# ChaissonLab/LRA

Hardware: AMD Instinct MI355X
Metric: aligned Gbp/s, 30 kb ONT vs GRCh38 (MapRead_lowacc end to end incl. SAM text), per job (higher is better)
Workload: dtype int32

## Files before the change

lra_amd/csrc/indel_refine.hip:

```cpp
#include "common.h"
#include "scan.h"
#include <algorithm>
#include <stdlib.h>

int lra_aog_launch_device(lra_ctx* ctx, int n, const char* d_qseq, const char* d_tseq, const uint64_t* d_q_off,
                          const int32_t* d_q_len, const uint64_t* d_t_off, const int32_t* d_t_len, const int32_t* d_k,
                          int m, int mm, int indel, int32_t* d_score, int32_t* d_nblocks, int32_t* d_blocks,
                          const uint64_t* d_block_off, int32_t* d_status);

namespace {

constexpr int BAD = -999999999;
constexpr int NEG = -2000000000;
enum { C_DIAG = 0, C_LEFT = 1, C_DOWN = 2, C_BOUND = 3, C_DELCLOSE = 4, C_INSCLOSE = 5, C_DONE = 6 };

__device__ __forceinline__ void wave_sync() {
  __builtin_amdgcn_fence(__ATOMIC_RELEASE, "workgroup");
  __builtin_amdgcn_wave_barrier();
  __builtin_amdgcn_fence(__ATOMIC_ACQUIRE, "workgroup");
}

__device__ __forceinline__ void wave_sync_lds() {
  __builtin_amdgcn_fence(__ATOMIC_RELEASE, "wavefront");
  __builtin_amdgcn_wave_barrier();
// ... 87 lines not shown
        qStart += advanced; tStart += advanced;
      }
      long ll = el;
      if (el > maxGap) {
        usedAlt = true;
        altQ = eq + maxGap; altT = et + maxGap; altL = el - maxGap;
        ll = maxGap;
        qPos = eq + maxGap; tPos = et + maxGap;
      }
      const long qEnd = eq + ll, tEnd = et + ll;
      const long tLen = tPos - tStart;
      const long tSeqLen = tEnd - tStart, qSeqLen = qEnd - qStart;
      const bool aog = (tSeqLen < k || qSeqLen < k);
      if (EMIT) {
        const uint64_t s = so + nseg;
        A.s_aln[s] = a; A.s_kind[s] = aog ? 1 : 0;
        A.s_qStart[s] = (int)qStart; A.s_tStart[s] = (int)tStart; A.s_qEnd[s] = (int)qEnd; A.s_tEnd[s] = (int)tEnd;
        A.s_b0[s] = (int)startBlock; A.s_b1[s] = (int)endBlock;
        A.s_first[3 * s] = (int)fq; A.s_first[3 * s + 1] = (int)ft; A.s_first[3 * s + 2] = (int)fl;
        A.s_lastLen[s] = (int)ll;
        A.s_rows[s] = aog ? 0 : (uint64_t)(tLen > 0 ? tLen : 0);
        A.s_isAog[s] = aog ? 1u : 0u;
        A.i_kind[io + nitem] = 1; A.i_data[3 * (io + nitem)] = (int)(nseg);
      }
      nitem++; nseg++;
    }
    if (!usedAlt) endBlock++;
    else { ovIdx = endBlock; ovQ = altQ; ovT = altT; ovL = altL; }
    startBlock = endBlock;
  }
  if (!EMIT) { A.a_nseg[a] = nseg; A.a_nitem[a] = nitem; A.a_status[a] = 0; }
}

struct __attribute__((aligned(16))) Row { int S, E; unsigned int C; int T; };

constexpr int CB = 32;
constexpr int MAXW = 1024;

struct BandArgs {
  uint64_t n_seg, n_task;
  const int32_t* s_aln; const int32_t* s_kind; const int32_t* s_qStart; const int32_t* s_qEnd; const int32_t* s_tStart;
  const int32_t* s_b0; const int32_t* s_b1; const int32_t* s_first; const int32_t* s_lastLen;
  const uint64_t* s_rows; const uint64_t* s_row_off;
  const int32_t* ab; const uint64_t* block_off;
  const char* tseq; const uint64_t* t_off;
  int k;
  Row* rows;
  uint64_t* s_cells; int32_t* s_status; int32_t* s_width; uint64_t* s_tmpcap;
  uint32_t* s_nchunk; const uint64_t* chunk_off; uint32_t* task_seg; int32_t* chunkT; int32_t* chunkQ;
};

struct SegBlocks {
  const int32_t* ab; long b0, b1; int fq, ft, fl, lastLen;
  __device__ __forceinline__ void get(long b, long& q, long& t, long& l) const {
    if (b == b0) { q = fq; t = ft; l = fl; }
    else { q = ab[3 * b]; t = ab[3 * b + 1]; l = (b == b1) ? lastLen : ab[3 * b + 2]; }
  }
};
__device__ __forceinline__ SegBlocks seg_blocks(const BandArgs& B, uint64_t s) {
  SegBlocks v;
  const int a = B.s_aln[s];
  v.ab = B.ab + 3 * (B.block_off[a] + 2 * (uint64_t)a);
  v.b0 = B.s_b0[s]; v.b1 = B.s_b1[s];
  v.fq = B.s_first[3 * s]; v.ft = B.s_first[3 * s + 1]; v.fl = B.s_first[3 * s + 2]; v.lastLen = B.s_lastLen[s];
  return v;
}
struct BlockStep { int bqGap, btGap; long blockLength, rows, advq; };
__device__ __forceinline__ BlockStep block_step(const SegBlocks& sb, long b, long bq, long bt, long bl, long& nq2, long& nt2, long& nl2) {
  BlockStep st; st.bqGap = 0; st.btGap = 0; st.blockLength = bl; nq2 = nt2 = nl2 = 0;
  if (b < sb.b1) {
    sb.get(b + 1, nq2, nt2, nl2);
    st.bqGap = (int)(nq2 - (bq + bl)); st.btGap = (int)(nt2 - (bt + bl));
    if (st.bqGap > 0 && st.btGap > 0) { int c = min(st.bqGap, st.btGap); st.bqGap -= c; st.btGap -= c; st.blockLength += c; }
  }
  const long body = st.blockLength > 0 ? st.blockLength : 0;
  st.rows = body + (st.btGap > st.bqGap && st.btGap > 0 ? st.btGap : 0);
  st.advq = body + (st.bqGap > st.btGap && st.bqGap > 0 ? st.bqGap : 0);
  return st;
}

// ... 109 lines not shown
      flush(tOff - k);
    }
    if (st.bqGap > st.btGap) {
      for (int qi = 0; qi < st.bqGap; qi++, q++)
        for (int ki = 0; ki < k; ki++) {
          if (tOff - ki >= 0 && tOff - ki < tLen) { if (RG(ringE, tOff - ki) < q) RG(ringE, tOff - ki) = (int)q; }
          if (tOff + ki < tLen) { int v = RG(ringS, tOff + ki); if (v == 0 || v > q) RG(ringS, tOff + ki) = (int)q; }
        }
    }
    if (st.btGap > st.bqGap) {
      for (int ti = 0; ti < st.btGap; ti++) {
        if (tOff >= tLen) { status |= 1; break; }
        const int e = (int)min(qEnd - 1, q + k);
        RG(ringS, tOff) = (int)max(q - k, qStart); RG(ringE, tOff) = e;
        if (e < eMin) eMin = e;
        if (sHi < tOff) sHi = tOff;
        tOff++;
        flush(tOff - k);
      }
    }
    bq = nq2; bt = nt2; bl = nl2;
  }
  if (lastChunk) for (long r = max(0L, tOff - k + 1); r < tLen; r++) flush(r);
#undef RG
  if (!multi) { if (tOff != tLen) status |= 1; B.s_status[s] = status; }
}

__global__ void __launch_bounds__(64) ir_band_scan(BandArgs B) {
  const uint64_t s = blockIdx.x;
  const int lane = threadIdx.x;
  if (B.s_kind[s] != 0) { if (lane == 0) { B.s_cells[s] = 0; B.s_status[s] = 0; B.s_width[s] = 0; B.s_tmpcap[s] = 0; } return; }
  int status = B.s_status[s];
  const long tLen = (long)B.s_rows[s];
  Row* rows = B.rows + B.s_row_off[s];
  unsigned long long cells = 0;
  int width = 0;
  if (!status && tLen > 0) {
    int run = 0x7fffffff;
    for (long base = ((tLen - 1) / 64) * 64; base >= 0; base -= 64) {
      const long r = base + lane;
      const int own = (r < tLen) ? rows[r].S : 0x7fffffff;
      int v = own;
      for (int d = 1; d < 64; d <<= 1) { int o = __shfl_down(v, d); if (lane + d < 64) v = min(v, o); }
      v = min(v, run);
      if (r < tLen && v != own) rows[r].S = v;
      run = __shfl(v, 0);
    }
    const int a = B.s_aln[s];
    const unsigned char* tb = (const unsigned char*)B.tseq + B.t_off[a] + B.s_tStart[s];
    int runE = -0x7fffffff;
    for (long base = 0; base < tLen; base += 64) {
      const long r = base + lane;
      Row w; w.S = 0; w.E = -0x7fffffff; w.C = 0; w.T = 0;
      if (r < tLen) w = rows[r];
      int e = w.E;
      for (int d = 1; d < 64; d <<= 1) { int o = __shfl_up(e, d); if (lane >= d) e = max(e, o); }
      e = max(e, runE);
      runE = __shfl(e, 63);
      int len = (r < tLen) ? e - w.S + 1 : 0;
      if (r < tLen) {
        if (len < 1 || w.S < 0) status |= 1;
        else if (len > MAXW) status |= 4;
        width = max(width, len);
      }
      const unsigned long long l = (unsigned long long)max(len, 0);
      unsigned long long inc = l;
      for (int d = 1; d < 64; d <<= 1) { unsigned long long o = __shfl_up(inc, d); if (lane >= d) inc += o; }
      if (r < tLen) { w.E = e; w.C = (unsigned int)(cells + inc - l); w.T = tb[r]; rows[r] = w; }
      cells += __shfl(inc, 63);
    }
    for (int o = 32; o > 0; o >>= 1) { status |= __shfl_xor(status, o); width = max(width, __shfl_xor(width, o)); }
  }
  if (lane == 0) {
    B.s_cells[s] = status ? 0 : cells;
    B.s_status[s] = status;
    B.s_width[s] = status ? 0 : width;
    B.s_tmpcap[s] = status ? 0 : (uint64_t)(tLen + ((long)B.s_qEnd[s] - B.s_qStart[s]) + 2);
  }
}

constexpr int FILL_BINS = 128;
template <bool EMIT>
__global__ void ir_classify(uint64_t n_seg, const int32_t* __restrict__ s_kind, const int32_t* __restrict__ s_status, const int32_t* __restrict__ s_width,
                            const uint64_t* __restrict__ s_rows, int* bins, uint32_t* list) {
  const uint64_t s = (uint64_t)blockIdx.x * blockDim.x + threadIdx.x;
  const int lane = threadIdx.x & 63;
  int bin = -1;
  if (s < n_seg && s_kind[s] == 0 && s_status[s] == 0) {
    const int w = s_width[s];
    const uint32_t r = (uint32_t)min((unsigned long long)s_rows[s], 0x7fffffffULL);
    bin = (w <= 16 ? 0 : w <= 32 ? 1 : w <= 64 ? 2 : 3) * 32 + (r ? __clz(r) : 31);
  }
  const unsigned long long below = (lane == 0) ? 0ULL : (~0ULL >> (64 - lane));
  unsigned long long todo = __ballot(bin >= 0);
  while (todo) {
    const int leader = __ffsll((long long)todo) - 1;
    const int b = __shfl(bin, leader);
    const unsigned long long m = __ballot(bin == b);
    int base = 0;
    if (lane == leader) base = atomicAdd(&bins[b], __popcll(m));
    base = __shfl(base, leader);
    if (EMIT && bin == b) list[base + __popcll(m & below)] = (uint32_t)s;
// ... 7 lines not shown
  const Row* rows;
  const char* qseq; const uint64_t* q_off; const int32_t* q_len;
  int match, mismatch, g;
  unsigned char* path;
  const uint32_t* list; int* cursor;
};

__device__ __forceinline__ bool is_bound(long row, int c, int len) { return c == len - 1 || (row > 0 && c == 0); }

__device__ __forceinline__ int shr1(int x, int fill) { return __builtin_amdgcn_update_dpp(fill, x, 0x138, 0xf, 0xf, false); }
template <int G>
__device__ __forceinline__ int scan_max(int w) {
  w = max(w, __builtin_amdgcn_update_dpp(NEG, w, 0x111, 0xf, 0xf, false));
  w = max(w, __builtin_amdgcn_update_dpp(NEG, w, 0x112, 0xf, 0xf, false));
  w = max(w, __builtin_amdgcn_update_dpp(NEG, w, 0x114, 0xf, 0xf, false));
  w = max(w, __builtin_amdgcn_update_dpp(NEG, w, 0x118, 0xf, 0xf, false));
  if (G >= 32) w = max(w, __builtin_amdgcn_update_dpp(NEG, w, 0x142, 0xa, 0xf, false));
  if (G >= 64) w = max(w, __builtin_amdgcn_update_dpp(NEG, w, 0x143, 0xc, 0xf, false));
  return w;
}

template <int G>
__global__ void __launch_bounds__(64) ir_fill(FillArgs F) {
  constexpr int GP = 64 / G;
  constexpr int CLS = (G == 16) ? 0 : (G == 32) ? 1 : 2;
  const int lane = threadIdx.x;
  const int c = lane % G, gbase = lane - c;
  const int g = F.g, go = 2 * F.g + 1;
  const long listEnd = F.cursor[4 + CLS];
  const uint32_t* list = F.list;
  long ti = -1, tLen = 0;
  const Row* rows = nullptr; const unsigned char* qb = nullptr; unsigned char* P = nullptr;
  long chunkBase = 0, qLast = 0;
  Row chunk; chunk.S = chunk.E = chunk.T = 0; chunk.C = 0;
  int W0 = 0, qlo = 0, qhi = 0, qnext = 0;
  int prevM = BAD, prevD = BAD, prevS = 0, prevLen = 0;
  bool done = false;
  auto ldq = [&](long idx) -> int { return qb[idx < qLast ? idx : qLast]; };
  while (true) {
    if (!done && ti < 0) {
      long x = 0;
      if (c == 0) x = atomicAdd(&F.cursor[CLS], 1);
      x = __shfl(x, gbase);
      if (x < listEnd) {
        const uint64_t s = list[x];
        const int a = F.s_aln[s];
        tLen = (long)F.s_rows[s];
        rows = F.rows + F.s_row_off[s];
        qb = (const unsigned char*)F.qseq + F.q_off[a];
        qLast = (long)F.q_len[a] - 1;
        P = F.path + F.s_cell_off[s];
        ti = 0; chunkBase = 0;
        if (c < tLen) chunk = rows[c];
        W0 = rows[0].S;
        qlo = ldq((long)W0 + c); qhi = ldq((long)W0 + G + c); qnext = ldq((long)W0 + 2 * G + c);
      } else done = true;
    }
    if (__ballot(!done) == 0ULL) break;
    if (!done && ti - chunkBase == G) { chunkBase = ti; if (ti + c < tLen) chunk = rows[ti + c]; }
    const int src = gbase + (int)((ti - chunkBase) & (G - 1));
    const int S = __shfl(chunk.S, src), E = __shfl(chunk.E, src), tch = __shfl(chunk.T, src);
    const unsigned int C = __shfl(chunk.C, src);
    while (!done && S - W0 >= G) { W0 += G; qlo = qhi; qhi = qnext; qnext = ldq((long)W0 + 2 * G + c); }
    const int j = S - W0 + c;
    const int q1 = __shfl(qlo, gbase + (j & (G - 1))), q2 = __shfl(qhi, gbase + (j & (G - 1)));
    const int qch = (j < G) ? q1 : q2;
    const int len = E - S + 1;
    const bool lastRow = (ti == tLen - 1);
    const int off = S - prevS;
    const bool interior = c >= 1 && (lastRow ? c <= len - 1 : c <= len - 2);
    const int srcA = c + off, srcD = srcA - 1;
    const bool aboveIn = srcA <= prevLen - 1;
    const int aM = __shfl(prevM, gbase + (srcA & (G - 1))), aD = __shfl(prevD, gbase + (srcA & (G - 1)));
    const int dM = shr1(aM, BAD);
    const bool okA = aboveIn && !is_bound(ti - 1, srcA, prevLen);
    const bool okD = aboveIn && srcD >= 0 && !is_bound(ti - 1, srcD, prevLen);
    const int dOpen = okA ? aM + go : BAD, dExt = okA ? aD : BAD;
    const int Dv = max(dOpen, dExt);
    const int delOpen = (Dv == dOpen) ? 1 : 0;
    const int mS = okD ? dM + (tch == qch ? F.match : F.mismatch) : BAD;
    const int dS = okA ? aM + g : BAD;
    const int V = interior ? max(mS, max(dS, Dv)) : NEG;
    const int W = scan_max<G>(V);
    int Wm1 = shr1(W, NEG), Vm1 = shr1(V, NEG);
    if (c == 0) { Wm1 = NEG; Vm1 = NEG; }
    const int Iv = max(BAD, go + Wm1);
    int M = max(max(BAD, V), max(Vm1 + g, go + Wm1));
    if (!interior) M = BAD;
    int Mleft = shr1(M, BAD);
    if (c <= 1) Mleft = BAD;
    const int iOpen = Mleft + go;
    const int insOpen = (Iv == iOpen) ? 1 : 0;
    const int iS = Mleft + g;
    int code;
    if (!interior) code = C_BOUND;
    else if (M == mS) code = C_DIAG;
    else if (M == iS) code = C_LEFT;
    else if (M == dS) code = C_DOWN;
    else if (M == Dv) code = C_DELCLOSE;
    else code = C_INSCLOSE;
    int outM = M, outD = interior ? Dv : BAD;
    unsigned char outB = (unsigned char)(code | (delOpen << 3) | (insOpen << 4));
    if (ti == 0) {
      const bool last0 = (c == len - 1) && (tLen > 1);
      outM = last0 ? BAD : (c == 0 ? 0 : c * g);
      outD = BAD;
      outB = (unsigned char)(last0 ? C_BOUND : (c == 0 ? C_DONE : C_LEFT));
    }
    if (!done) {
      if (c < len) P[C + c] = outB;
      prevM = outM; prevD = outD; prevS = S; prevLen = len;
      ti++;
      if (ti == tLen) ti = -1;
    }
  }
}


__global__ void __launch_bounds__(64) ir_fill_wide(FillArgs F) {
  __shared__ int sM[2][MAXW + 64], sD[2][MAXW + 64];
  const int lane = threadIdx.x;
  const int g = F.g, go = 2 * F.g + 1;
  const long listEnd = F.cursor[4 + 3];
  while (true) {
    long x = 0;
    if (lane == 0) x = atomicAdd(&F.cursor[3], 1);
    x = (long)(((unsigned long long)(unsigned)__builtin_amdgcn_readfirstlane((int)((unsigned long long)x >> 32)) << 32) | (unsigned)__builtin_amdgcn_readfirstlane((int)(x & 0xffffffffL)));
    if (x >= listEnd) break;
    const uint64_t s = F.list[x];
    const int a = F.s_aln[s];
    const long tLen = (long)F.s_rows[s];
    const Row* rows = F.rows + F.s_row_off[s];
    const unsigned char* qb = (const unsigned char*)F.qseq + F.q_off[a];
    const long qLast = (long)F.q_len[a] - 1;
    unsigned char* P = F.path + F.s_cell_off[s];
    int prevS = 0, prevLen = 0;
    for (long ti = 0; ti < tLen; ti++) {
      const Row rw = rows[ti];
      const int S = rw.S, len = rw.E - rw.S + 1, tch = rw.T;
      const unsigned int C = rw.C;
      const bool lastRow = (ti == tLen - 1);
      const int off = S - prevS;
      const int cur = (int)(ti & 1), prv = cur ^ 1;
      int carryW = NEG, carryV = NEG, carryM = BAD;
      for (int base = 0; base < len; base += 64) {
        const int c = base + lane;
        int outM, outD; unsigned char outB;
        if (ti == 0) {
          const bool last0 = (c == len - 1) && (tLen > 1);
          outM = last0 ? BAD : (c == 0 ? 0 : c * g);
          outD = BAD;
          outB = (unsigned char)(last0 ? C_BOUND : (c == 0 ? C_DONE : C_LEFT));
        } else {
          const long qi = (long)S + c;
          const int qch = qb[qi < qLast ? qi : qLast];
          const bool interior = c >= 1 && (lastRow ? c <= len - 1 : c <= len - 2);
          const int srcA = c + off, srcD = srcA - 1;
          const bool aboveIn = srcA <= prevLen - 1;
          const bool inA = srcA >= 0 && srcA < prevLen, inD = srcD >= 0 && srcD < prevLen;
          const int aM = inA ? sM[prv][srcA] : BAD, aD = inA ? sD[prv][srcA] : BAD;
          const int dM = inD ? sM[prv][srcD] : BAD;
          const bool okA = aboveIn && !is_bound(ti - 1, srcA, prevLen);
          const bool okD = aboveIn && srcD >= 0 && !is_bound(ti - 1, srcD, prevLen);
          const int dOpen = okA ? aM + go : BAD, dExt = okA ? aD : BAD;
          const int Dv = max(dOpen, dExt);
          const int delOpen = (Dv == dOpen) ? 1 : 0;
          const int mS = okD ? dM + (tch == qch ? F.match : F.mismatch) : BAD;
          const int dS = okA ? aM + g : BAD;
          const int V = interior ? max(mS, max(dS, Dv)) : NEG;
          const int W = max(scan_max<64>(V), carryW);
          int Wm1 = shr1(W, NEG), Vm1 = shr1(V, NEG);
          if (lane == 0) { Wm1 = carryW; Vm1 = carryV; }
          if (c == 0) { Wm1 = NEG; Vm1 = NEG; }
          const int Iv = max(BAD, go + Wm1);
          int M = max(max(BAD, V), max(Vm1 + g, go + Wm1));
          if (!interior) M = BAD;
          int Mleft = shr1(M, BAD);
          if (lane == 0) Mleft = carryM;
          if (c <= 1) Mleft = BAD;
          const int iOpen = Mleft + go;
          const int insOpen = (Iv == iOpen) ? 1 : 0;
          const int iS = Mleft + g;
          int code;
          if (!interior) code = C_BOUND;
          else if (M == mS) code = C_DIAG;
          else if (M == iS) code = C_LEFT;
          else if (M == dS) code = C_DOWN;
          else if (M == Dv) code = C_DELCLOSE;
          else code = C_INSCLOSE;
          outM = M; outD = interior ? Dv : BAD;
          outB = (unsigned char)(code | (delOpen << 3) | (insOpen << 4));
          carryW = __shfl(W, 63); carryV = __shfl(V, 63); carryM = __shfl(M, 63);
        }
        if (c < len) { P[C + c] = outB; sM[cur][c] = outM; sD[cur][c] = outD; }
      }
      wave_sync_lds();
      prevS = S; prevLen = len;
    }
  }
}

template <int N>
__device__ __forceinline__ int ror(int x) { return __builtin_amdgcn_update_dpp(0, x, 0x120 + N, 0xf, 0xf, true); }
__device__ __forceinline__ int pin(int x) { asm volatile("" : "+v"(x)); return x; }
__device__ __forceinline__ int ring_scan_max(int w, int d) {
  { const int t = pin(max(w, ror<1>(w))); w = (d >= 1) ? t : w; }
  { const int t = pin(max(w, ror<2>(w))); w = (d >= 2) ? t : w; }
  { const int t = pin(max(w, ror<4>(w))); w = (d >= 4) ? t : w; }
  { const int t = pin(max(w, ror<8>(w))); w = (d >= 8) ? t : w; }
  return w;
}
template <int NP>
__global__ void __launch_bounds__(64) ir_fill_cols(FillArgs F) {
  constexpr int G = 16;
  constexpr int CLS = NP - 1;
  const int lane = threadIdx.x;
  const int c = lane % G, gbase = lane - c;
  const int g = F.g, go = 2 * F.g + 1;
  const long listEnd = F.cursor[4 + CLS];
  const uint32_t* list = F.list;
  long ti = -1, tLen = 0;
  const Row* rows = nullptr; const unsigned char* qb = nullptr; unsigned char* P = nullptr;
  long qLast = 0;
  __shared__ Row s_chunk[64];
  long chunkBase = 0;
  Row chunk; chunk.S = chunk.E = chunk.T = 0; chunk.C = 0;
  int K0 = 0, q0 = 0, q1 = 0, q2 = 0, q3 = 0;
  int pM[NP], pD[NP], prevS = 0, prevLen = 0;
  for (int p = 0; p < NP; p++) { pM[p] = BAD; pD[p] = BAD; }
  bool done = false;
  auto ldq = [&](long idx) -> int { return qb[idx < qLast ? idx : qLast]; };
  while (true) {
    if (!done && ti < 0) {
      long x = 0;
      if (c == 0) x = atomicAdd(&F.cursor[CLS], 1);
      x = __shfl(x, gbase);
      if (x < listEnd) {
        const uint64_t s = list[x];
        const int a = F.s_aln[s];
        tLen = (long)F.s_rows[s];
        rows = F.rows + F.s_row_off[s];
        qb = (const unsigned char*)F.qseq + F.q_off[a];
        qLast = (long)F.q_len[a] - 1;
        P = F.path + F.s_cell_off[s];
        ti = 0; chunkBase = -G;
        if (c < tLen) chunk = rows[c];
        K0 = rows[0].S >> 4;
        const long b = 16L * K0 + c;
        q0 = ldq(b); q1 = ldq(b + G); q2 = ldq(b + 2 * G); q3 = ldq(b + 3 * G);
      } else done = true;
    }
    if (__ballot(!done) == 0ULL) break;
    if (!done && ti - chunkBase == G) {
      chunkBase = ti;
      s_chunk[lane] = chunk;
      wave_sync_lds();
      if (ti + G + c < tLen) chunk = rows[ti + G + c];
    }
    const Row rw = s_chunk[gbase + (int)((ti - chunkBase) & (G - 1))];
    const int S = rw.S, E = rw.E, tch = rw.T;
    const unsigned int C = rw.C;
    if (!done && (S >> 4) != K0) {
      const int adv = (S >> 4) - K0;
      K0 = S >> 4;
      const long b = 16L * K0 + c;
      if (adv == 1) { q0 = q1; q1 = q2; q2 = q3; }
      else { q0 = ldq(b); q1 = ldq(b + G); q2 = ldq(b + 2 * G); }
      q3 = ldq(b + 3 * G);
    }
    const int len = E - S + 1;
    const bool lastRow = (ti == tLen - 1);
    const int off = S - prevS;
    const int d = (c - S) & (G - 1);
    const bool head = (d == 0);
    const bool lo = c >= (S & (G - 1));
    int nM[NP], nD[NP];
    for (int p = 0; p < NP; p++) { nM[p] = BAD; nD[p] = BAD; }
    int cW = NEG, cV = NEG, cM = BAD, cA = BAD;
    for (int p = 0; p < NP; p++) {
      if (p == 1 && len <= G) break;
      const int cc = d + G * p;
      const int qch = (p == 0) ? (lo ? q0 : q1) : (lo ? q1 : q2);
      const bool interior = cc >= 1 && (lastRow ? cc <= len - 1 : cc <= len - 2);
      const int srcA = cc + off, srcD = srcA - 1;
      const bool aboveIn = srcA <= prevLen - 1;
      const int aM = (NP > 1 && srcA >= G) ? pM[NP - 1] : pM[0];
      const int aD = (NP > 1 && srcA >= G) ? pD[NP - 1] : pD[0];
      const int rA = pin(ror<1>(aM));
      const int dM = (p == 1 && head) ? cA : rA;
      const bool okA = aboveIn && !is_bound(ti - 1, srcA, prevLen);
      const bool okD = aboveIn && srcD >= 0 && !is_bound(ti - 1, srcD, prevLen);
      const int dOpen = okA ? aM + go : BAD, dExt = okA ? aD : BAD;
      const int Dv = max(dOpen, dExt);
      const int delOpen = (Dv == dOpen) ? 1 : 0;
      const int mS = okD ? dM + (tch == qch ? F.match : F.mismatch) : BAD;
      const int dS = okA ? aM + g : BAD;
      const int V = interior ? max(mS, max(dS, Dv)) : NEG;
      const int W = ring_scan_max((p == 1 && head) ? max(V, cW) : V, d);
      const int rW = pin(ror<1>(W)), rV = pin(ror<1>(V));
      const int Wm1 = head ? cW : rW, Vm1 = head ? cV : rV;
      const int Iv = max(BAD, go + Wm1);
      int M = max(max(BAD, V), max(Vm1 + g, go + Wm1));
      if (!interior) M = BAD;
      const int rM = pin(ror<1>(M));
      int Mleft = head ? cM : rM;
      if (cc <= 1) Mleft = BAD;
      const int iOpen = Mleft + go;
      const int insOpen = (Iv == iOpen) ? 1 : 0;
      const int iS = Mleft + g;
      int code;
      if (!interior) code = C_BOUND;
      else if (M == mS) code = C_DIAG;
      else if (M == iS) code = C_LEFT;
      else if (M == dS) code = C_DOWN;
      else if (M == Dv) code = C_DELCLOSE;
      else code = C_INSCLOSE;
      int outM = M, outD = interior ? Dv : BAD;
      unsigned char outB = (unsigned char)(code | (delOpen << 3) | (insOpen << 4));
      if (ti == 0) {
        const bool last0 = (cc == len - 1) && (tLen > 1);
        outM = last0 ? BAD : (cc == 0 ? 0 : cc * g);
        outD = BAD;
        outB = (unsigned char)(last0 ? C_BOUND : (cc == 0 ? C_DONE : C_LEFT));
      }
      if (!done && cc < len) P[C + cc] = outB;
      nM[p] = outM; nD[p] = outD;
      if (NP > 1 && p == 0) { cW = rW; cV = rV; cM = rM; cA = rA; }
    }
    if (!done) {
      for (int p = 0; p < NP; p++) { pM[p] = nM[p]; pD[p] = nD[p]; }
      prevS = S; prevLen = len;
      ti++;
      if (ti == tLen) ti = -1;
    }
  }
}

struct TraceArgs {
  uint64_t n_seg;
  const int32_t* s_kind; const int32_t* s_tStart; const uint64_t* s_rows; const uint64_t* s_row_off;
  const uint64_t* s_cells; const uint64_t* s_cell_off; int32_t* s_status;
  const Row* rows;
  const unsigned char* path;
  uint32_t* s_nblk;
  const uint64_t* s_tmp_off; int32_t* tmp_blocks;
};

constexpr int TW_ROWS = 128, TW_PATH = 4096;
__global__ void __launch_bounds__(64) ir_trace_wave(TraceArgs T) {
  __shared__ Row s_rows[TW_ROWS];
  __shared__ __attribute__((aligned(16))) unsigned char s_path[TW_PATH + 16];
  const int lane = threadIdx.x;
  const uint64_t s = blockIdx.x;
  if (s >= T.n_seg) return;
  if (T.s_kind[s] != 0) return;
  if (T.s_status[s] != 0) { if (lane == 0) T.s_nblk[s] = 0; return; }
  const long tLen = (long)T.s_rows[s];
  const Row* rows = T.rows + T.s_row_off[s];
  const unsigned char* P = T.path + T.s_cell_off[s];
  int32_t* ob = T.tmp_blocks + 3 * T.s_tmp_off[s];
  const long cap = (long)(T.s_tmp_off[s + 1] - T.s_tmp_off[s]);
  long ti = tLen - 1;
  long rBase = 0, wLo = 1, wHi = 0; unsigned pBase = 0;
  auto stage = [&](long at) {
    wave_sync();
    wHi = at; rBase = max(0L, at - TW_ROWS + 1);
    for (long x = lane; x <= at - rBase; x += 64) s_rows[x] = rows[rBase + x];
    wave_sync();
    const Row last = s_rows[at - rBase];
    const unsigned end = last.C + (unsigned)max(last.E - last.S + 1, 0);
    long lo = rBase, hi = at;
    while (lo < hi) { const long mid = (lo + hi) >> 1; if (end - s_rows[mid - rBase].C <= (unsigned)TW_PATH) hi = mid; else lo = mid + 1; }
    wLo = lo; pBase = s_rows[lo - rBase].C;
    const unsigned nbytes = min(end - pBase, (unsigned)TW_PATH);
    const unsigned char* start = P + pBase;
    const unsigned delta = (unsigned)((uintptr_t)start & 15);
    const uint4* a16 = (const uint4*)(start - delta);
    const unsigned full = (delta + nbytes) >> 4;
    for (unsigned x = lane; x < full; x += 64) ((uint4*)s_path)[x] = a16[x];
    for (unsigned x = (full << 4) + lane; x < delta + nbytes; x += 64) s_path[x] = (start - delta)[x];
    pBase -= delta;
    wave_sync();
  };
  stage(ti);
  Row rw = s_rows[ti - rBase];
  int qa = rw.E;
  int mat = 0;
  int bad = 0;
  long nblk = 0;
  long q = (long)rw.E + 1, t = (long)T.s_tStart[s] + tLen;
  int curKind = -1, pending = 0;
  long dlen = 0;
  long steps = 0;
  const long step_cap = 4 * (long)T.s_cells[s] + 64;
  auto emit_block = [&]() {
    if (nblk < cap) { if (lane == 0) { ob[3 * nblk] = (int)q; ob[3 * nblk + 1] = (int)t; ob[3 * nblk + 2] = (int)dlen; } } else bad = 1;
    nblk++;
  };
  auto op = [&](int kind, long times) {
    if (kind != curKind) {
      if (curKind == -1 && kind == 0) { pending = 1; dlen = 0; }
      if (kind != 0) {
        if (pending) emit_block();
        pending = 1; dlen = 0;
      }
      curKind = kind;
    }
    if (kind == 0) { dlen += times; q -= times; t -= times; }
    else if (kind == 1) q -= times;
    else t -= times;
  };
  while (true) {
    if (ti < wLo || ti > wHi) stage(ti);
    rw = s_rows[ti - rBase];
    if (mat == 0) {
      const long tl = ti - lane;
      bool fast = false;
      if (tl >= wLo && tl >= 1) {
        const Row r = s_rows[tl - rBase];
        const int c = (qa - lane) - r.S;
        if (c >= 0 && c <= r.E - r.S) fast = (s_path[r.C - pBase + (unsigned)c] & 7) == C_DIAG;
      }
      const unsigned long long nf = ~__ballot(fast);
      const int f = nf ? __ffsll((long long)nf) - 1 : 64;
      if (f > 0) {
        steps += f;
        if (steps > step_cap) { bad = 1; break; }
        op(0, f); ti -= f; qa -= f;
        continue;
      }
    }
    const int c = qa - rw.S;
    if (c < 0 || c > rw.E - rw.S) { bad = 1; break; }
    if (ti == 0 && c == 0) break;
    if (++steps > step_cap) { bad = 1; break; }
    const unsigned char pb = s_path[rw.C - pBase + (unsigned)c];
    long nti = ti;
    if (mat == 0) {
      const int code = pb & 7;
      if (code == C_DELCLOSE) mat = 1;
      else if (code == C_INSCLOSE) mat = 2;
      else if (code == C_DIAG) { op(0, 1); nti = ti - 1; qa--; }
      else if (code == C_LEFT) { op(1, 1); qa--; }
      else if (code == C_DOWN) { op(2, 1); nti = ti - 1; }
      else { bad = 1; break; }
    } else if (mat == 1) {
      op(2, 1);
      mat = ((pb >> 3) & 1) ? 0 : 1;
      nti = ti - 1;
    } else {
      op(1, 1);
      mat = ((pb >> 4) & 1) ? 0 : 2;
      qa--;
    }
    if (nti != ti) {
      if (nti < 0) { bad = 1; break; }
      ti = nti;
    }
  }
  if (!bad) {
    op(0, 1);
    if (pending) emit_block();
  }
  if (lane == 0) {
    if (bad) T.s_status[s] |= 2;
    T.s_nblk[s] = bad ? 0 : (uint32_t)nblk;
  }
}

// ... 158 lines not shown
  add(capSeg, 8); add(capSeg, 4); add(capSeg, 8); add(capSeg, 4); add(capSeg, 4); add(capSeg, 4); add(capSeg + 1, 8);
  add(capSeg, 4); add(capSeg, 4); add(capSeg, 4);
  add(capSeg, 4); add(capSeg + 1, 8);
  char* baseA = (char*)lra_scratch(ctx, 2, needA + 4096);
  if (!baseA) return LRA_ERR_NOMEM;
  Arena ar{baseA, needA + 4096, 0};
  A.ab = ar.get<int32_t>(3 * nBk);
  A.s_aln = ar.get<int32_t>(capSeg); A.s_kind = ar.get<int32_t>(capSeg); A.s_qStart = ar.get<int32_t>(capSeg); A.s_tStart = ar.get<int32_t>(capSeg);
  A.s_qEnd = ar.get<int32_t>(capSeg); A.s_tEnd = ar.get<int32_t>(capSeg); A.s_b0 = ar.get<int32_t>(capSeg); A.s_b1 = ar.get<int32_t>(capSeg);
  A.s_first = ar.get<int32_t>(3 * capSeg); A.s_lastLen = ar.get<int32_t>(capSeg); A.s_rows = ar.get<uint64_t>(capSeg); A.s_isAog = ar.get<uint32_t>(capSeg);
  uint64_t* s_row_off = ar.get<uint64_t>(capSeg + 1); uint64_t* s_aog_off = ar.get<uint64_t>(capSeg + 1);
  uint64_t* s_cells = ar.get<uint64_t>(capSeg); uint64_t* s_cell_off = ar.get<uint64_t>(capSeg + 1); int32_t* s_status = ar.get<int32_t>(capSeg);
  uint32_t* s_nblk = ar.get<uint32_t>(capSeg); int32_t* s_width = ar.get<int32_t>(capSeg); uint64_t* s_tmpcap = ar.get<uint64_t>(capSeg);
  uint64_t* s_tmp_off = ar.get<uint64_t>(capSeg + 1); uint32_t* s_aog_idx = ar.get<uint32_t>(capSeg); uint64_t* s_out_off = ar.get<uint64_t>(capSeg + 1);
  uint32_t* fill_lists = ar.get<uint32_t>(capSeg); int* fill_counts = ar.get<int>(FILL_BINS + 8);
  A.i_kind = ar.get<int32_t>(capItem); A.i_data = ar.get<int32_t>(3 * capItem);
  int32_t* i_aln = ar.get<int32_t>(capItem); uint32_t* i_count = ar.get<uint32_t>(capItem); uint64_t* i_out_off = ar.get<uint64_t>(capItem + 1);
  uint64_t* p_q_off = ar.get<uint64_t>(capSeg); int32_t* p_q_len = ar.get<int32_t>(capSeg); uint64_t* p_t_off = ar.get<uint64_t>(capSeg);
  int32_t* p_t_len = ar.get<int32_t>(capSeg); int32_t* p_k = ar.get<int32_t>(capSeg); uint32_t* p_cap = ar.get<uint32_t>(capSeg);
  uint64_t* p_block_off = ar.get<uint64_t>(capSeg + 1);
  int32_t* p_score = ar.get<int32_t>(capSeg); int32_t* p_nblocks = ar.get<int32_t>(capSeg); int32_t* p_status = ar.get<int32_t>(capSeg);
  uint32_t* s_nchunk = ar.get<uint32_t>(capSeg); uint64_t* chunk_off = ar.get<uint64_t>(capSeg + 1);
  if (!chunk_off) return lra_set_err(ctx, LRA_ERR_NOMEM, "arena accounting");
  lra_time_begin(ctx, "ir_segment");
  hipLaunchKernelGGL(ir_segment<true>, dim3(nbA), dim3(64), 0, st, A);
  lra_time_end(ctx);
  hipLaunchKernelGGL(ir_item_aln, dim3((n_aln + 255) / 256), dim3(256), 0, st, n_aln, item_off, i_aln);
  uint64_t n_rows = 0, n_aog = 0, n_cells = 0;
  const int32_t* tmp_blocks = nullptr;
  if (n_seg) {
    scan(ctx, (long)n_seg, A.s_rows, s_row_off);
    scan(ctx, (long)n_seg, A.s_isAog, s_aog_off);
    if (d2h(ctx, &n_rows, s_row_off + n_seg, 8) || d2h(ctx, &n_aog, s_aog_off + n_seg, 8)) return LRA_ERR_HIP;
    Row* rows = (Row*)lra_ensure(ctx, 0, (n_rows + 1) * sizeof(Row));
    if (!rows) return LRA_ERR_NOMEM;
    BandArgs B;
    B.n_seg = n_seg; B.s_aln = A.s_aln; B.s_kind = A.s_kind; B.s_qStart = A.s_qStart; B.s_qEnd = A.s_qEnd; B.s_tStart = A.s_tStart;
    B.s_b0 = A.s_b0; B.s_b1 = A.s_b1; B.s_first = A.s_first; B.s_lastLen = A.s_lastLen; B.s_rows = A.s_rows; B.s_row_off = s_row_off;
    B.ab = A.ab; B.block_off = d_block_off; B.tseq = d_tseq; B.t_off = d_t_off; B.k = refine_band; B.rows = rows;
    B.s_cells = s_cells; B.s_status = s_status; B.s_width = s_width; B.s_tmpcap = s_tmpcap;
    const unsigned gridL = (unsigned)((n_seg + 63) / 64);
    const unsigned gridS = (unsigned)((n_seg + 255) / 256);
    lra_time_begin(ctx, "ir_band");
    B.s_nchunk = s_nchunk; B.chunk_off = chunk_off; B.n_task = 0; B.task_seg = nullptr; B.chunkT = nullptr; B.chunkQ = nullptr;
    hipLaunchKernelGGL(ir_band_nchunk, dim3(gridS), dim3(256), 0, st, B);
    scan(ctx, (long)n_seg, s_nchunk, chunk_off);
    uint64_t n_task = 0;
    if (d2h(ctx, &n_task, chunk_off + n_seg, 8)) return LRA_ERR_HIP;
    uint32_t* task_seg = (uint32_t*)lra_ensure(ctx, 54, (n_task + 1) * 4);
    int32_t* chunk_tq = (int32_t*)lra_ensure(ctx, 55, (n_task + 1) * 8);
    if (!task_seg || !chunk_tq) return LRA_ERR_NOMEM;
    B.n_task = n_task; B.task_seg = task_seg; B.chunkT = chunk_tq; B.chunkQ = chunk_tq + n_task + 1;
    hipLaunchKernelGGL(ir_band_tasks, dim3(gridS), dim3(256), 0, st, B);
    hipLaunchKernelGGL(ir_band_prep, dim3((unsigned)n_seg), dim3(64), 0, st, B);
    if (n_task) {
      const unsigned gridT = (unsigned)((n_task + 63) / 64);
      if (refine_band <= 8) hipLaunchKernelGGL(ir_band_chunk<16>, dim3(gridT), dim3(64), 0, st, B);
      else if (refine_band <= 32) hipLaunchKernelGGL(ir_band_chunk<64>, dim3(gridT), dim3(64), 0, st, B);
      else hipLaunchKernelGGL(ir_band_chunk<128>, dim3(gridT), dim3(64), 0, st, B);
    }
    hipLaunchKernelGGL(ir_band_scan, dim3((unsigned)n_seg), dim3(64), 0, st, B);
    lra_time_end(ctx);
    scan(ctx, (long)n_seg, s_cells, s_cell_off);
    scan(ctx, (long)n_seg, s_tmpcap, s_tmp_off);
    uint64_t n_tmp = 0;
    if (d2h(ctx, &n_cells, s_cell_off + n_seg, 8) || d2h(ctx, &n_tmp, s_tmp_off + n_seg, 8)) return LRA_ERR_HIP;
    const size_t pathBytes = (n_cells + 256 + 255) & ~(size_t)255;
    unsigned char* path = (unsigned char*)lra_ensure(ctx, 12, pathBytes + (n_tmp + 1) * 12 + 256);
    if (!path) return LRA_ERR_NOMEM;
    int32_t* tmpb = (int32_t*)(path + pathBytes);
    tmp_blocks = tmpb;
    int h_bins[FILL_BINS], h_start[FILL_BINS], h_cursor[8] = {0, 0, 0, 0, 0, 0, 0, 0};
    LRA_HIP_CHECK(ctx, hipMemsetAsync(fill_counts, 0, FILL_BINS * 4, st));
    hipLaunchKernelGGL(ir_classify<false>, dim3((unsigned)((n_seg + 255) / 256)), dim3(256), 0, st, n_seg, A.s_kind, s_status, s_width, A.s_rows, fill_counts, fill_lists);
    if (d2h(ctx, h_bins, fill_counts, FILL_BINS * 4)) return LRA_ERR_HIP;
    { int run = 0; for (int b = 0; b < FILL_BINS; b++) { h_start[b] = run; run += h_bins[b]; if ((b & 31) == 0) h_cursor[b / 32] = h_start[b]; if ((b & 31) == 31) h_cursor[4 + b / 32] = run; } }
    LRA_HIP_CHECK(ctx, hipMemcpyAsync(fill_counts, h_start, FILL_BINS * 4, hipMemcpyHostToDevice, st));
    hipLaunchKernelGGL(ir_classify<true>, dim3((unsigned)((n_seg + 255) / 256)), dim3(256), 0, st, n_seg, A.s_kind, s_status, s_width, A.s_rows, fill_counts, fill_lists);
    int* fill_cursor = fill_counts + FILL_BINS;
    LRA_HIP_CHECK(ctx, hipMemcpyAsync(fill_cursor, h_cursor, 32, hipMemcpyHostToDevice, st));
    FillArgs F;
    F.n_seg = n_seg; F.s_aln = A.s_aln; F.s_rows = A.s_rows; F.s_row_off = s_row_off; F.s_cell_off = s_cell_off; F.rows = rows;
    F.qseq = d_qseq; F.q_off = d_q_off; F.q_len = d_q_len; F.match = match; F.mismatch = mismatch; F.g = indel; F.path = path;
    F.list = fill_lists; F.cursor = fill_cursor;
    const unsigned cap_grid = (unsigned)ctx->num_cu * 32;
    if (getenv("LRA_IR_DBG")) {
      const int hc[4] = {h_cursor[4] - h_cursor[0], h_cursor[5] - h_cursor[1], h_cursor[6] - h_cursor[2], h_cursor[7] - h_cursor[3]};
      fprintf(stderr, "[ir] n_seg %llu n_rows %llu n_cells %llu n_task %llu n_item %llu fill classes 16/32/64/wide: %d %d %d %d\n",
              (unsigned long long)n_seg, (unsigned long long)n_rows, (unsigned long long)n_cells, (unsigned long long)n_task,
              (unsigned long long)n_item, hc[0], hc[1], hc[2], hc[3]);
    }
    lra_time_begin(ctx, "ir_fill");
    const uint64_t n16 = (uint64_t)(h_cursor[4] - h_cursor[0]), n32 = (uint64_t)(h_cursor[5] - h_cursor[1]), n64 = (uint64_t)(h_cursor[6] - h_cursor[2]);
    const uint64_t nWide = (uint64_t)(h_cursor[7] - h_cursor[3]);
    if (n16) hipLaunchKernelGGL(ir_fill_cols<1>, dim3((unsigned)std::min<uint64_t>((n16 + 3) / 4, cap_grid)), dim3(64), 0, lra_side_fork(ctx, 1), F);
    if (n64) hipLaunchKernelGGL(ir_fill<64>, dim3((unsigned)std::min<uint64_t>(n64, cap_grid)), dim3(64), 0, lra_side_fork(ctx, 2), F);
    if (nWide) hipLaunchKernelGGL(ir_fill_wide, dim3((unsigned)std::min<uint64_t>(nWide, cap_grid)), dim3(64), 0, lra_side_fork(ctx, 3), F);
    if (n32) hipLaunchKernelGGL(ir_fill_cols<2>, dim3((unsigned)std::min<uint64_t>((n32 + 3) / 4, cap_grid)), dim3(64), 0, st, F);
    if (n16) lra_side_join(ctx, 1);
    if (n64) lra_side_join(ctx, 2);
    if (nWide) lra_side_join(ctx, 3);
    lra_time_end(ctx);
    TraceArgs T;
    T.n_seg = n_seg; T.s_kind = A.s_kind; T.s_tStart = A.s_tStart; T.s_rows = A.s_rows; T.s_row_off = s_row_off;
    T.s_cells = s_cells; T.s_cell_off = s_cell_off; T.s_status = s_status; T.rows = rows; T.path = path;
    T.s_nblk = s_nblk; T.s_tmp_off = s_tmp_off; T.tmp_blocks = tmpb;
    lra_time_begin(ctx, "ir_trace");
    hipLaunchKernelGGL(ir_trace_wave, dim3((unsigned)n_seg), dim3(64), 0, st, T);
    lra_time_end(ctx);
    if (n_aog) {
      hipLaunchKernelGGL(ir_aog_setup, dim3((unsigned)((n_seg + 255) / 256)), dim3(256), 0, st, n_seg, A.s_kind, A.s_aln, s_aog_off, A.s_qStart,
                         A.s_tStart, A.s_qEnd, A.s_tEnd, d_q_off, d_t_off, refine_band, s_aog_idx, p_q_off, p_q_len, p_t_off, p_t_len, p_k, p_cap);
      scan(ctx, (long)n_aog, p_cap, p_block_off);
      uint64_t aog_cap = 0;
      if (d2h(ctx, &aog_cap, p_block_off + n_aog, 8)) return LRA_ERR_HIP;
      if (aog_cap * 12 + 64 > ctx->aux_bytes) {
        if (ctx->aux) (void)hipFree(ctx->aux);
        ctx->aux = nullptr; ctx->aux_bytes = 0;
        size_t want = aog_cap * 12 + aog_cap * 3 + 4096;
        if (hipMalloc(&ctx->aux, want) != hipSuccess) return lra_set_err(ctx, LRA_ERR_NOMEM, "aog block buffer");
        ctx->aux_bytes = want;
      }
      int rc = lra_aog_launch_device(ctx, (int)n_aog, d_qseq, d_tseq, p_q_off, p_q_len, p_t_off, p_t_len, p_k, match, mismatch, indel, p_score,
                                     p_nblocks, (int32_t*)ctx->aux, p_block_off, p_status);
      if (rc) return rc;
    }
  }
  hipLaunchKernelGGL(ir_item_counts, dim3((unsigned)((n_item + 255) / 256)), dim3(256), 0, st, n_item, A.i_kind, A.i_data, i_aln, seg_off, A.s_kind,
                     s_nblk, s_aog_idx, p_nblocks, i_count);
  scan(ctx, (long)n_item, i_count, i_out_off);
  uint64_t n_out = 0;
  if (d2h(ctx, &n_out, i_out_off + n_item, 8)) return LRA_ERR_HIP;
  if ((n_out + 1) * 12 > ctx->out_bytes) {
    if (ctx->out_buf) (void)hipFree(ctx->out_buf);
    ctx->out_buf = nullptr; ctx->out_bytes = 0;
    size_t want = (n_out + 1) * 12 + (n_out + 1) * 3 + 4096;
    if (hipMalloc(&ctx->out_buf, want) != hipSuccess) return lra_set_err(ctx, LRA_ERR_NOMEM, "refined block buffer");
    ctx->out_bytes = want;
// ... 20 lines not shown
```

lra_amd/csrc/scan.h:

```cpp
#pragma once
#include "common.h"

namespace { namespace lra_scan_detail {

constexpr int NT = 256;

template <typename CT>
__global__ void __launch_bounds__(NT) tile_sum(long n, long tile, const CT* __restrict__ c, uint64_t* __restrict__ part) {
  __shared__ uint64_t red[NT / 64];
  const long lo = (long)blockIdx.x * tile, hi = (lo + tile < n) ? lo + tile : n;
  uint64_t s = 0;
  for (long i = lo + threadIdx.x; i < hi; i += NT) s += (uint64_t)c[i];
  for (int o = 32; o > 0; o >>= 1) s += __shfl_xor(s, o);
  if ((threadIdx.x & 63) == 0) red[threadIdx.x >> 6] = s;
  __syncthreads();
  if (threadIdx.x == 0) { uint64_t t = 0; for (int w = 0; w < NT / 64; w++) t += red[w]; part[blockIdx.x] = t; }
}

static __global__ void __launch_bounds__(1024) part_scan(long nb, uint64_t* part) {
  __shared__ uint64_t sh[1024];
  const int t = threadIdx.x;
  const long per = (nb + 1023) / 1024;
  const long lo = (long)t * per < nb ? (long)t * per : nb, hi = lo + per < nb ? lo + per : nb;
  uint64_t s = 0;
  for (long i = lo; i < hi; i++) s += part[i];
  sh[t] = s;
  __syncthreads();
  for (int d = 1; d < 1024; d <<= 1) {
    uint64_t v = (t >= d) ? sh[t - d] : 0;
    __syncthreads();
    sh[t] += v;
    __syncthreads();
  }
  uint64_t run = (t == 0) ? 0 : sh[t - 1];
// ... 46 lines not shown
```

Measured before the change: 1.085.

## Pack band rows to 8 bytes and derive cell offsets via checkpoints and DPP scans

Shrinks the per-row band record from 16 bytes to 8 by packing length and target base into one word. Per-row cell offsets are no longer stored: fill kernels accumulate them on the fly, and trace rebuilds them from a checkpoint stored every 64 rows. The wave min/max/sum scans switch from shuffle loops to DPP row operations and are unrolled four tiles deep to cut memory traffic and shuffle latency. This adds a re-scan in the trace staging path, and clamping the stored length to 16 bits depends on MAXW limiting row widths.

```diff
diff --git a/lra_amd/csrc/indel_refine.hip b/lra_amd/csrc/indel_refine.hip
--- a/lra_amd/csrc/indel_refine.hip
+++ b/lra_amd/csrc/indel_refine.hip
@@ -143,7 +143,13 @@
   if (!EMIT) { A.a_nseg[a] = nseg; A.a_nitem[a] = nitem; A.a_status[a] = 0; }
 }
 
-struct __attribute__((aligned(16))) Row { int S, E; unsigned int C; int T; };
+struct __attribute__((aligned(8))) Row {
+  int S; unsigned int lt;
+  __device__ __forceinline__ int len() const { return (int)(lt & 0xffffu) + 1; }
+  __device__ __forceinline__ int T() const { return (int)((lt >> 16) & 0xffu); }
+};
+constexpr int CK_ROWS = 64;
+__device__ __forceinline__ uint64_t ck_off(uint64_t row_off, uint64_t s) { return (row_off >> 6) + s; }
 
 constexpr int CB = 32;
 constexpr int MAXW = 1024;
@@ -156,7 +162,7 @@
   const int32_t* ab; const uint64_t* block_off;
   const char* tseq; const uint64_t* t_off;
   int k;
-  Row* rows;
+  Row* rows; uint32_t* ck;
   uint64_t* s_cells; int32_t* s_status; int32_t* s_width; uint64_t* s_tmpcap;
   uint32_t* s_nchunk; const uint64_t* chunk_off; uint32_t* task_seg; int32_t* chunkT; int32_t* chunkQ;
 };
@@ -332,42 +338,60 @@
   if (B.s_kind[s] != 0) { if (lane == 0) { B.s_cells[s] = 0; B.s_status[s] = 0; B.s_width[s] = 0; B.s_tmpcap[s] = 0; } return; }
   int status = B.s_status[s];
   const long tLen = (long)B.s_rows[s];
-  Row* rows = B.rows + B.s_row_off[s];
+  const uint64_t ro = B.s_row_off[s];
+  Row* rows = B.rows + ro;
+  int2* raw = (int2*)rows;
+  uint32_t* ck = B.ck + ck_off(ro, s);
   unsigned long long cells = 0;
   int width = 0;
+  constexpr int SCAN_U = 4;
   if (!status && tLen > 0) {
     int run = 0x7fffffff;
-    for (long base = ((tLen - 1) / 64) * 64; base >= 0; base -= 64) {
-      const long r = base + lane;
-      const int own = (r < tLen) ? rows[r].S : 0x7fffffff;
-      int v = own;
-      for (int d = 1; d < 64; d <<= 1) { int o = __shfl_down(v, d); if (lane + d < 64) v = min(v, o); }
-      v = min(v, run);
-      if (r < tLen && v != own) rows[r].S = v;
-      run = __shfl(v, 0);
-    }
+    for (long tile = (tLen - 1) / 64; tile >= 0; tile -= SCAN_U) {
+      int own[SCAN_U];
+#pragma unroll
+      for (int u = 0; u < SCAN_U; u++) {
+        const long r = (tile - u) * 64 + 63 - lane;
+        own[u] = (r >= 0 && r < tLen) ? raw[r].x : 0x7fffffff;
+      }
+#pragma unroll
+      for (int u = 0; u < SCAN_U; u++) {
+        const long r = (tile - u) * 64 + 63 - lane;
+        const int v = min(wave_incl_min(own[u]), run);
+        if (r >= 0 && r < tLen && v != own[u]) raw[r].x = v;
+        run = __builtin_amdgcn_readlane(v, 63);
+      }
+    }
+    wave_sync();
     const int a = B.s_aln[s];
     const unsigned char* tb = (const unsigned char*)B.tseq + B.t_off[a] + B.s_tStart[s];
     int runE = -0x7fffffff;
-    for (long base = 0; base < tLen; base += 64) {
-      const long r = base + lane;
-      Row w; w.S = 0; w.E = -0x7fffffff; w.C = 0; w.T = 0;
-      if (r < tLen) w = rows[r];
-      int e = w.E;
-      for (int d = 1; d < 64; d <<= 1) { int o = __shfl_up(e, d); if (lane >= d) e = max(e, o); }
-      e = max(e, runE);
-      runE = __shfl(e, 63);
-      int len = (r < tLen) ? e - w.S + 1 : 0;
-      if (r < tLen) {
-        if (len < 1 || w.S < 0) status |= 1;
-        else if (len > MAXW) status |= 4;
-        width = max(width, len);
-      }
-      const unsigned long long l = (unsigned long long)max(len, 0);
-      unsigned long long inc = l;
-      for (int d = 1; d < 64; d <<= 1) { unsigned long long o = __shfl_up(inc, d); if (lane >= d) inc += o; }
-      if (r < tLen) { w.E = e; w.C = (unsigned int)(cells + inc - l); w.T = tb[r]; rows[r] = w; }
-      cells += __shfl(inc, 63);
+    for (long base = 0; base < tLen; base += 64 * SCAN_U) {
+      int2 w[SCAN_U]; unsigned int tch[SCAN_U];
+#pragma unroll
+      for (int u = 0; u < SCAN_U; u++) {
+        const long r = base + 64 * u + lane;
+        w[u].x = 0; w[u].y = -0x7fffffff; tch[u] = 0;
+        if (r < tLen) { w[u] = raw[r]; tch[u] = tb[r]; }
+      }
+#pragma unroll
+      for (int u = 0; u < SCAN_U; u++) {
+        const long r = base + 64 * u + lane;
+        if (base + 64 * u >= tLen) break;
+        const int e = max(wave_incl_max(w[u].y), runE);
+        runE = __builtin_amdgcn_readlane(e, 63);
+        const int len = (r < tLen) ? e - w[u].x + 1 : 0;
+        if (r < tLen) {
+          if (len < 1 || w[u].x < 0) status |= 1;
+          else if (len > MAXW) status |= 4;
+          width = max(width, len);
+        }
+        const int l = min(max(len, 0), MAXW);
+        const int inc = wave_incl_add(l);
+        if (lane == 0) ck[(base >> 6) + u] = (uint32_t)cells;
+        if (r < tLen) { Row o; o.S = w[u].x; o.lt = (unsigned int)max(l - 1, 0) | (tch[u] << 16); rows[r] = o; }
+        cells += (unsigned int)__builtin_amdgcn_readlane(inc, 63);
+      }
     }
     for (int o = 32; o > 0; o >>= 1) { status |= __shfl_xor(status, o); width = max(width, __shfl_xor(width, o)); }
   }
@@ -441,7 +465,8 @@
   long ti = -1, tLen = 0;
   const Row* rows = nullptr; const unsigned char* qb = nullptr; unsigned char* P = nullptr;
   long chunkBase = 0, qLast = 0;
-  Row chunk; chunk.S = chunk.E = chunk.T = 0; chunk.C = 0;
+  Row chunk; chunk.S = 0; chunk.lt = 0;
+  unsigned int C = 0;
   int W0 = 0, qlo = 0, qhi = 0, qnext = 0;
   int prevM = BAD, prevD = BAD, prevS = 0, prevLen = 0;
   bool done = false;
@@ -459,7 +484,7 @@
         qb = (const unsigned char*)F.qseq + F.q_off[a];
         qLast = (long)F.q_len[a] - 1;
         P = F.path + F.s_cell_off[s];
-        ti = 0; chunkBase = 0;
+        ti = 0; chunkBase = 0; C = 0;
         if (c < tLen) chunk = rows[c];
         W0 = rows[0].S;
         qlo = ldq((long)W0 + c); qhi = ldq((long)W0 + G + c); qnext = ldq((long)W0 + 2 * G + c);
@@ -468,13 +493,14 @@
     if (__ballot(!done) == 0ULL) break;
     if (!done && ti - chunkBase == G) { chunkBase = ti; if (ti + c < tLen) chunk = rows[ti + c]; }
     const int src = gbase + (int)((ti - chunkBase) & (G - 1));
-    const int S = __shfl(chunk.S, src), E = __shfl(chunk.E, src), tch = __shfl(chunk.T, src);
-    const unsigned int C = __shfl(chunk.C, src);
+    const int S = __shfl(chunk.S, src);
+    const unsigned int lt = (unsigned int)__shfl((int)chunk.lt, src);
+    const int tch = (int)((lt >> 16) & 0xffu);
     while (!done && S - W0 >= G) { W0 += G; qlo = qhi; qhi = qnext; qnext = ldq((long)W0 + 2 * G + c); }
     const int j = S - W0 + c;
     const int q1 = __shfl(qlo, gbase + (j & (G - 1))), q2 = __shfl(qhi, gbase + (j & (G - 1)));
     const int qch = (j < G) ? q1 : q2;
-    const int len = E - S + 1;
+    const int len = (int)(lt & 0xffffu) + 1;
     const bool lastRow = (ti == tLen - 1);
     const int off = S - prevS;
     const bool interior = c >= 1 && (lastRow ? c <= len - 1 : c <= len - 2);
@@ -519,6 +545,7 @@
     if (!done) {
       if (c < len) P[C + c] = outB;
       prevM = outM; prevD = outD; prevS = S; prevLen = len;
+      C += (unsigned int)len;
       ti++;
       if (ti == tLen) ti = -1;
     }
@@ -544,10 +571,10 @@
     const long qLast = (long)F.q_len[a] - 1;
     unsigned char* P = F.path + F.s_cell_off[s];
     int prevS = 0, prevLen = 0;
+    unsigned int C = 0;
     for (long ti = 0; ti < tLen; ti++) {
       const Row rw = rows[ti];
-      const int S = rw.S, len = rw.E - rw.S + 1, tch = rw.T;
-      const unsigned int C = rw.C;
+      const int S = rw.S, len = rw.len(), tch = rw.T();
       const bool lastRow = (ti == tLen - 1);
       const int off = S - prevS;
       const int cur = (int)(ti & 1), prv = cur ^ 1;
@@ -605,6 +632,7 @@
       }
       wave_sync_lds();
       prevS = S; prevLen = len;
+      C += (unsigned int)len;
     }
   }
 }
@@ -633,7 +661,8 @@
   long qLast = 0;
   __shared__ Row s_chunk[64];
   long chunkBase = 0;
-  Row chunk; chunk.S = chunk.E = chunk.T = 0; chunk.C = 0;
+  Row chunk; chunk.S = 0; chunk.lt = 0;
+  unsigned int C = 0;
   int K0 = 0, q0 = 0, q1 = 0, q2 = 0, q3 = 0;
   int pM[NP], pD[NP], prevS = 0, prevLen = 0;
   for (int p = 0; p < NP; p++) { pM[p] = BAD; pD[p] = BAD; }
@@ -652,7 +681,7 @@
         qb = (const unsigned char*)F.qseq + F.q_off[a];
         qLast = (long)F.q_len[a] - 1;
         P = F.path + F.s_cell_off[s];
-        ti = 0; chunkBase = -G;
+        ti = 0; chunkBase = -G; C = 0;
         if (c < tLen) chunk = rows[c];
         K0 = rows[0].S >> 4;
         const long b = 16L * K0 + c;
@@ -667,8 +696,7 @@
       if (ti + G + c < tLen) chunk = rows[ti + G + c];
     }
     const Row rw = s_chunk[gbase + (int)((ti - chunkBase) & (G - 1))];
-    const int S = rw.S, E = rw.E, tch = rw.T;
-    const unsigned int C = rw.C;
+    const int S = rw.S, tch = rw.T();
     if (!done && (S >> 4) != K0) {
       const int adv = (S >> 4) - K0;
       K0 = S >> 4;
@@ -677,7 +705,7 @@
       else { q0 = ldq(b); q1 = ldq(b + G); q2 = ldq(b + 2 * G); }
       q3 = ldq(b + 3 * G);
     }
-    const int len = E - S + 1;
+    const int len = rw.len();
     const bool lastRow = (ti == tLen - 1);
     const int off = S - prevS;
     const int d = (c - S) & (G - 1);
@@ -739,6 +767,7 @@
     if (!done) {
       for (int p = 0; p < NP; p++) { pM[p] = nM[p]; pD[p] = nD[p]; }
       prevS = S; prevLen = len;
+      C += (unsigned int)len;
       ti++;
       if (ti == tLen) ti = -1;
     }
@@ -749,7 +778,7 @@
   uint64_t n_seg;
   const int32_t* s_kind; const int32_t* s_tStart; const uint64_t* s_rows; const uint64_t* s_row_off;
   const uint64_t* s_cells; const uint64_t* s_cell_off; int32_t* s_status;
-  const Row* rows;
+  const Row* rows; const uint32_t* ck;
   const unsigned char* path;
   uint32_t* s_nblk;
   const uint64_t* s_tmp_off; int32_t* tmp_blocks;
@@ -758,6 +787,7 @@
 constexpr int TW_ROWS = 128, TW_PATH = 4096;
 __global__ void __launch_bounds__(64) ir_trace_wave(TraceArgs T) {
   __shared__ Row s_rows[TW_ROWS];
+  __shared__ unsigned int s_C[TW_ROWS];
   __shared__ __attribute__((aligned(16))) unsigned char s_path[TW_PATH + 16];
   const int lane = threadIdx.x;
   const uint64_t s = blockIdx.x;
@@ -766,6 +796,7 @@
   if (T.s_status[s] != 0) { if (lane == 0) T.s_nblk[s] = 0; return; }
   const long tLen = (long)T.s_rows[s];
   const Row* rows = T.rows + T.s_row_off[s];
+  const uint32_t* ck = T.ck + ck_off(T.s_row_off[s], s);
   const unsigned char* P = T.path + T.s_cell_off[s];
   int32_t* ob = T.tmp_blocks + 3 * T.s_tmp_off[s];
   const long cap = (long)(T.s_tmp_off[s + 1] - T.s_tmp_off[s]);
@@ -774,13 +805,28 @@
   auto stage = [&](long at) {
     wave_sync();
     wHi = at; rBase = max(0L, at - TW_ROWS + 1);
-    for (long x = lane; x <= at - rBase; x += 64) s_rows[x] = rows[rBase + x];
+    const long aBase = rBase & ~(long)(CK_ROWS - 1);
+    Row w[3];
+#pragma unroll
+    for (int u = 0; u < 3; u++) {
+      const long r = aBase + 64 * u + lane;
+      w[u].S = 0; w[u].lt = 0;
+      if (r <= at) w[u] = rows[r];
+    }
+    unsigned end = ck[aBase / CK_ROWS];
+#pragma unroll
+    for (int u = 0; u < 3; u++) {
+      const long r = aBase + 64 * u + lane;
+      if (aBase + 64 * u > at) break;
+      const int len = (r <= at) ? w[u].len() : 0;
+      const int inc = wave_incl_add(len);
+      if (r >= rBase && r <= at) { s_rows[r - rBase] = w[u]; s_C[r - rBase] = end + (unsigned)(inc - len); }
+      end += (unsigned)__builtin_amdgcn_readlane(inc, 63);
+    }
     wave_sync();
-    const Row last = s_rows[at - rBase];
-    const unsigned end = last.C + (unsigned)max(last.E - last.S + 1, 0);
     long lo = rBase, hi = at;
-    while (lo < hi) { const long mid = (lo + hi) >> 1; if (end - s_rows[mid - rBase].C <= (unsigned)TW_PATH) hi = mid; else lo = mid + 1; }
-    wLo = lo; pBase = s_rows[lo - rBase].C;
+    while (lo < hi) { const long mid = (lo + hi) >> 1; if (end - s_C[mid - rBase] <= (unsigned)TW_PATH) hi = mid; else lo = mid + 1; }
+    wLo = lo; pBase = s_C[lo - rBase];
     const unsigned nbytes = min(end - pBase, (unsigned)TW_PATH);
     const unsigned char* start = P + pBase;
     const unsigned delta = (unsigned)((uintptr_t)start & 15);
@@ -793,11 +839,11 @@
   };
   stage(ti);
   Row rw = s_rows[ti - rBase];
-  int qa = rw.E;
+  int qa = rw.S + rw.len() - 1;
   int mat = 0;
   int bad = 0;
   long nblk = 0;
-  long q = (long)rw.E + 1, t = (long)T.s_tStart[s] + tLen;
+  long q = (long)qa + 1, t = (long)T.s_tStart[s] + tLen;
   int curKind = -1, pending = 0;
   long dlen = 0;
   long steps = 0;
@@ -828,7 +874,7 @@
       if (tl >= wLo && tl >= 1) {
         const Row r = s_rows[tl - rBase];
         const int c = (qa - lane) - r.S;
-        if (c >= 0 && c <= r.E - r.S) fast = (s_path[r.C - pBase + (unsigned)c] & 7) == C_DIAG;
+        if (c >= 0 && c < r.len()) fast = (s_path[s_C[tl - rBase] - pBase + (unsigned)c] & 7) == C_DIAG;
       }
       const unsigned long long nf = ~__ballot(fast);
       const int f = nf ? __ffsll((long long)nf) - 1 : 64;
@@ -840,10 +886,10 @@
       }
     }
     const int c = qa - rw.S;
-    if (c < 0 || c > rw.E - rw.S) { bad = 1; break; }
+    if (c < 0 || c >= rw.len()) { bad = 1; break; }
     if (ti == 0 && c == 0) break;
     if (++steps > step_cap) { bad = 1; break; }
-    const unsigned char pb = s_path[rw.C - pBase + (unsigned)c];
+    const unsigned char pb = s_path[s_C[ti - rBase] - pBase + (unsigned)c];
     long nti = ti;
     if (mat == 0) {
       const int code = pb & 7;
@@ -1068,12 +1114,14 @@
     scan(ctx, (long)n_seg, A.s_rows, s_row_off);
     scan(ctx, (long)n_seg, A.s_isAog, s_aog_off);
     if (d2h(ctx, &n_rows, s_row_off + n_seg, 8) || d2h(ctx, &n_aog, s_aog_off + n_seg, 8)) return LRA_ERR_HIP;
-    Row* rows = (Row*)lra_ensure(ctx, 0, (n_rows + 1) * sizeof(Row));
+    const size_t rowBytes = ((n_rows + 1) * sizeof(Row) + 255) & ~(size_t)255;
+    Row* rows = (Row*)lra_ensure(ctx, 0, rowBytes + (n_rows / CK_ROWS + n_seg + 2) * sizeof(uint32_t));
     if (!rows) return LRA_ERR_NOMEM;
+    uint32_t* ck = (uint32_t*)((char*)rows + rowBytes);
     BandArgs B;
     B.n_seg = n_seg; B.s_aln = A.s_aln; B.s_kind = A.s_kind; B.s_qStart = A.s_qStart; B.s_qEnd = A.s_qEnd; B.s_tStart = A.s_tStart;
     B.s_b0 = A.s_b0; B.s_b1 = A.s_b1; B.s_first = A.s_first; B.s_lastLen = A.s_lastLen; B.s_rows = A.s_rows; B.s_row_off = s_row_off;
-    B.ab = A.ab; B.block_off = d_block_off; B.tseq = d_tseq; B.t_off = d_t_off; B.k = refine_band; B.rows = rows;
+    B.ab = A.ab; B.block_off = d_block_off; B.tseq = d_tseq; B.t_off = d_t_off; B.k = refine_band; B.rows = rows; B.ck = ck;
     B.s_cells = s_cells; B.s_status = s_status; B.s_width = s_width; B.s_tmpcap = s_tmpcap;
     const unsigned gridL = (unsigned)((n_seg + 63) / 64);
     const unsigned gridS = (unsigned)((n_seg + 255) / 256);
@@ -1139,7 +1187,7 @@
     lra_time_end(ctx);
     TraceArgs T;
     T.n_seg = n_seg; T.s_kind = A.s_kind; T.s_tStart = A.s_tStart; T.s_rows = A.s_rows; T.s_row_off = s_row_off;
-    T.s_cells = s_cells; T.s_cell_off = s_cell_off; T.s_status = s_status; T.rows = rows; T.path = path;
+    T.s_cells = s_cells; T.s_cell_off = s_cell_off; T.s_status = s_status; T.rows = rows; T.ck = ck; T.path = path;
     T.s_nblk = s_nblk; T.s_tmp_off = s_tmp_off; T.tmp_blocks = tmpb;
     lra_time_begin(ctx, "ir_trace");
     hipLaunchKernelGGL(ir_trace_wave, dim3((unsigned)n_seg), dim3(64), 0, st, T);
diff --git a/lra_amd/csrc/scan.h b/lra_amd/csrc/scan.h
--- a/lra_amd/csrc/scan.h
+++ b/lra_amd/csrc/scan.h
@@ -1,5 +1,21 @@
 #pragma once
 #include "common.h"
+
+namespace {
+#define LRA_DPP_SCAN(OP_, ident_)                                                                  \
+  v = OP_(v, __builtin_amdgcn_update_dpp((ident_), v, 0x111, 0xf, 0xf, false));     \
+  v = OP_(v, __builtin_amdgcn_update_dpp((ident_), v, 0x112, 0xf, 0xf, false));     \
+  v = OP_(v, __builtin_amdgcn_update_dpp((ident_), v, 0x114, 0xf, 0xf, false));     \
+  v = OP_(v, __builtin_amdgcn_update_dpp((ident_), v, 0x118, 0xf, 0xf, false));     \
+  v = OP_(v, __builtin_amdgcn_update_dpp((ident_), v, 0x142, 0xa, 0xf, false));  \
+  v = OP_(v, __builtin_amdgcn_update_dpp((ident_), v, 0x143, 0xc, 0xf, false));
+#define LRA_SCAN_ADD(a_, b_) ((a_) + (b_))
+__device__ __forceinline__ int wave_incl_add(int v) { LRA_DPP_SCAN(LRA_SCAN_ADD, 0) return v; }
+__device__ __forceinline__ int wave_incl_max(int v) { LRA_DPP_SCAN(max, -0x7fffffff - 1) return v; }
+__device__ __forceinline__ int wave_incl_min(int v) { LRA_DPP_SCAN(min, 0x7fffffff) return v; }
+#undef LRA_SCAN_ADD
+#undef LRA_DPP_SCAN
+}
 
 namespace { namespace lra_scan_detail {
 
```

Result: no change. 1.085, median of 4 (-0.0%).
